# BoxLib-Codes/VARDEN

Hardware: AMD Instinct MI355X
Metric: cells*steps/sec on advance_timestep (higher is better)
Workload: dtype f64; 1 GPU; 3D 256x256x256 single-level variable-density bubble, 1 box(es) of 256^3, MAC+HG projection each step (BASELINE.json configs[1]); parallelism=single GPU, cells=16777216

## Files before the change

### varden_amd/csrc/mg_nd.hip

```cpp
#include "vdn_dev.h"
#include "mg_stop.h"
#include "krylov_wg.h"
#include "krylov_grid.h"
#include <tuple>
#include <algorithm>

struct NLev {
  int n[3]; int PX, PY; long sz;
  double f[3];
  double *phi, *tmp, *b, *res, *sig;
  int dirlo[3], dirhi[3];
  int per[3];
};
DEVI long nidx(const NLev &L, int i, int j, int k) { return (long)(i + 16) + (long)L.PX * ((long)(j + 1) + (long)L.PY * (long)(k + 1)); }
DEVI bool nd_is_dir(const NLev &L, int i, int j, int k) {
  return (i == 0 && L.dirlo[0]) || (i == L.n[0] && L.dirhi[0]) || (j == 0 && L.dirlo[1]) || (j == L.n[1] && L.dirhi[1]) ||
         (k == 0 && L.dirlo[2]) || (k == L.n[2] && L.dirhi[2]);
}
DEVI bool nd_is_shell(const NLev &L, int i, int j, int k, int hm) {
  return ((hm & 1) && i == 0) || ((hm & 2) && i == L.n[0]) || ((hm & 4) && j == 0) || ((hm & 8) && j == L.n[1]) ||
         ((hm & 16) && k == 0) || ((hm & 32) && k == L.n[2]);
}

struct NdW { double w0, w1, w2, w3, w4, w5, w6, w7; int iso; };
DEVI NdW nd_weights(const double f[3]) {
  const double fx = f[0], fy = f[1], fz = f[2];
  const double F = fx + fy + fz;
  NdW W;
  W.w0 = 4.0 * F;
  W.w1 = -4.0 * fx + 2.0 * fy + 2.0 * fz;
  W.w2 = 2.0 * fx - 4.0 * fy + 2.0 * fz;
  W.w3 = -2.0 * fx - 2.0 * fy + fz;
  W.w4 = 2.0 * fx + 2.0 * fy - 4.0 * fz;
  W.w5 = -2.0 * fx + fy - 2.0 * fz;
  W.w6 = fx - 2.0 * fy - 2.0 * fz;
  W.w7 = -F;
// ... 488 lines not shown
  const long sy = C.PX, sz = (long)C.PX * C.PY;
  const double *__restrict__ cp = C.phi;
  long c0 = nidx(C, c00 + (i >> 1), c01 + (j >> 1), c02 + (k0 >> 1));
  double a00 = cp[c0], a10 = cp[c0 + 1], a01 = cp[c0 + sy], a11 = cp[c0 + sy + 1];
  const bool dir_ij = (i == 0 && F.dirlo[0]) || (i == F.n[0] && F.dirhi[0]) || (j == 0 && F.dirlo[1]) || (j == F.n[1] && F.dirhi[1]);
  const double w0 = 1.0 / (double)((1 + oi) * (1 + oj)), w1 = 1.0 / (double)((1 + oi) * (1 + oj) * 2);
  for (int k = k0; k <= k1; k += 2) {
    const double b00 = cp[c0 + sz], b10 = cp[c0 + sz + 1], b01 = cp[c0 + sz + sy], b11 = cp[c0 + sz + sy + 1];
    const long f = nidx(F, i, j, k);
    const double pe = F.phi[f];
    const bool odd_in = k + 1 <= k1;
    const long f2 = f + (long)F.PX * F.PY;
    const double po = odd_in ? F.phi[f2] : 0.0;
    double s = 0.0;
    s = s + a00;
    s = oi ? s + a10 : s;
    s = oj ? s + a01 : s;
    s = (oi && oj) ? s + a11 : s;
    double t = s;
    t = t + b00;
    t = oi ? t + b10 : t;
    t = oj ? t + b01 : t;
    t = (oi && oj) ? t + b11 : t;
    if (!(dir_ij || (k == 0 && F.dirlo[2]) || (k == F.n[2] && F.dirhi[2]))) F.phi[f] = pe + s * w0;
    if (odd_in && !(dir_ij || (k + 1 == F.n[2] && F.dirhi[2]))) F.phi[f2] = po + t * w1;
    a00 = b00; a10 = b10; a01 = b01; a11 = b11; c0 += sz;
  }
}
static void nd_launch_prolong(const NLev &F, const NLev &C, int c00, int c01, int c02) {
  const int nzp = F.n[2] + 1;
  const int kchunk = nzp > 64 ? 16 : (nzp > 16 ? 8 : 2);
  hipLaunchKernelGGL(kk_nd_prolong_m, dim3((F.n[0] + 64) / 64, (F.n[1] + 4) / 4, (nzp + kchunk - 1) / kchunk), dim3(64, 4, 1), 0, ctx().stream, F, C, c00, c01, c02, kchunk);
}
__global__ void kk_nd_coarsen_sigma(NLev F, NLev C) {
  const int i = blockIdx.x * blockDim.x + threadIdx.x;
  const int j = blockIdx.y * blockDim.y + threadIdx.y;
  const int k = blockIdx.z;
  if (i >= C.n[0] || j >= C.n[1] || k >= C.n[2]) return;
  const long sy = F.PX, sz = (long)F.PX * F.PY;
  const long f = nidx(F, 2 * i, 2 * j, 2 * k);
  double s = 0.0;
  #pragma unroll
  for (int c = 0; c < 2; c++)
    #pragma unroll
    for (int b = 0; b < 2; b++)
      #pragma unroll
      for (int a = 0; a < 2; a++) s = s + F.sig[f + a + b * sy + c * sz];
  C.sig[nidx(C, i, j, k)] = s * 0.125;
}

__global__ void __launch_bounds__(1024) kk_nd_bottom(NLev L, double *a, double *b, int nsweeps, double omega, double om1 = 0.0, double om2 = 0.0, int nsp = 0) {
  const int ex = L.n[0] + 3, ey = L.n[1] + 3, ez = L.n[2] + 3;
  const int nx = L.n[0] + 1, ny = L.n[1] + 1, nz = L.n[2] + 1;
  double *src = a, *dst = b;
  for (int s = 0; s < nsweeps; s++) {
    for (int t = threadIdx.x; t < ex * ey * ez; t += blockDim.x) {
      const int i = t % ex - 1, j = (t / ex) % ey - 1, k = t / (ex * ey) - 1;
      int q[3] = { i, j, k }, sidx[3] = { i, j, k }; bool g = false, zero = false;
      for (int d = 0; d < 3; d++) {
        if (L.per[d]) { if (q[d] < 0) { sidx[d] = q[d] + L.n[d]; g = true; } else if (q[d] >= L.n[d]) { sidx[d] = q[d] - L.n[d]; g = true; } }
        else if (q[d] < 0 || q[d] > L.n[d]) { g = true; zero = true; }
      }
      if (g) src[nidx(L, i, j, k)] = zero ? 0.0 : src[nidx(L, sidx[0], sidx[1], sidx[2])];
    }
    __syncthreads();
    for (int t = threadIdx.x; t < nx * ny * nz; t += blockDim.x) {
// ... 326 lines not shown
  G.rev = 0;
  return G;
}
static bool nd_wide_level(const NLev &L) { return sw().nd_pair && L.n[0] >= 127; }
static bool nd_wide_even_level(const NLev &L) { return nd_wide_level(L) && L.n[0] % 2 == 0 && L.n[1] % 2 == 0 && L.n[2] % 2 == 0; }
template <int MODE> static void nd_launch_march(const NLev &L, const double *phi, double *out, double *nrm, int shell_later = 0, int rev = 0, const NLev *pro = nullptr) {
  const int nzp = L.n[2] + 1;
  const int tiles = ((L.n[0] + 62) / 62) * ((L.n[1] + 4) / 4);
  int kchunk = nzp;
  while (kchunk > 8 && tiles * ((nzp + kchunk - 1) / kchunk) < 2048) kchunk = (kchunk + 1) / 2;
  const int nch = (nzp + kchunk - 1) / kchunk;
  if (nd_wide_level(L)) {
    const int rows = 4;
    const bool use_rem = true; const int minwg = 2048, kc_env = 0;
    NdPairGrid G = nd_pair_grid(L, rows, nzp, use_rem, minwg, kc_env);
    G.rev = sw().nd_rev ? rev : 0;
    if (MODE == 0 && pro) {
      const NdCoarse C{ pro->phi, pro->PX, pro->PY, pro->n[0] };
      hipLaunchKernelGGL((kk_nd_march_pair<0, 4, 1>), dim3(G.nmain + G.gyr * G.gz), NBLK, 0, ctx().stream, L, phi, out, nd_cur_omega(), G, nrm, shell_later, C);
      return;
    }
    hipLaunchKernelGGL((kk_nd_march_pair<MODE, 4>), dim3(G.nmain + G.gyr * G.gz), NBLK, 0, ctx().stream, L, phi, out, nd_cur_omega(), G, nrm, shell_later, NdCoarse{ nullptr, 0, 0, 0 });
    return;
  }
  REQUIRE(!pro, "nodal multigrid: the prolonging sweep is the paired march's");
  hipLaunchKernelGGL(kk_nd_march<MODE>, dim3((L.n[0] + 62) / 62, (L.n[1] + 4) / 4, nch), NBLK, 0, ctx().stream, L, phi, out, nd_cur_omega(), kchunk, nrm, shell_later);
}

struct NBox { NLev L; int lo[3]; int hmask = 63; XPlan *hA = nullptr, *hB = nullptr; double *A = nullptr, *B = nullptr; };
struct NDLev { std::vector<NBox> boxes; XPlan *halo_A = nullptr, *halo_B = nullptr, *halo_res = nullptr, *halo_sig = nullptr; int ng[3]; bool flip = false; bool single_box = false; int per[3] = {0, 0, 0};
               int rev = 0;
               bool res_restricted = false;  };
struct NDMG {
  std::vector<NDLev> dlev; std::vector<NLev> tail; int per[3]; double *d_nrm; unsigned pro_levels = 0;
  MgGather g_nodes, g_cells; GBox *d_gb = nullptr;
  double *sendbuf = nullptr, *recvbuf = nullptr;
  MgKrylov kry;
};

__global__ void kk_nd_zero_shell(NLev L, double *a0, double *a1, double *a2) {
  const int u = (int)(blockIdx.x * blockDim.x + threadIdx.x) - 1, v = (int)(blockIdx.y * blockDim.y + threadIdx.y) - 1;
  const int face = blockIdx.z, d = face >> 1, side = face & 1;
  const int da = d == 0 ? 1 : 0, db = d == 2 ? 1 : 2;
  if (u > L.n[da] + 1 || v > L.n[db] + 1) return;
  int q[3]; q[d] = side ? L.n[d] + 1 : -1; q[da] = u; q[db] = v;
  const long c = nidx(L, q[0], q[1], q[2]);
  a0[c] = 0.0; if (a1) a1[c] = 0.0; if (a2) a2[c] = 0.0;
}
static NLev nd_alloc_lev(const int n[3], const double h[3]) {
  NLev L;
  for (int d = 0; d < 3; d++) { L.n[d] = n[d]; L.f[d] = 1.0 / (36.0 * (h[d] * h[d])); L.dirlo[d] = L.dirhi[d] = L.per[d] = 0; }
  L.PX = ((n[0] + 18 + 15) / 16) * 16; L.PY = n[1] + 3; L.sz = (long)L.PX * L.PY * (n[2] + 3);
  double *base = (double *)arena_alloc(sizeof(double) * L.sz * 5);
  L.phi = base; L.tmp = base + L.sz; L.b = base + 2 * L.sz; L.res = base + 3 * L.sz; L.sig = base + 4 * L.sz;
  if (sw().nd_lean && (long)(n[0] + 1) * (n[1] + 1) * (n[2] + 1) >= (1L << 21)) {
    const int m = std::max(n[0], std::max(n[1], n[2])) + 3;
    hipLaunchKernelGGL(kk_nd_zero_shell, dim3((m + 63) / 64, (m + 3) / 4, 6), dim3(64, 4, 1), 0, ctx().stream, L, L.phi, L.tmp, L.res);
    HIPCHK(hipMemsetAsync(L.sig, 0, sizeof(double) * L.sz, ctx().stream));
  } else HIPCHK(hipMemsetAsync(base, 0, sizeof(double) * L.sz * 5, ctx().stream));
  return L;
}
static FV nd_view(const NLev &L, double *p, const int lo[3], int extra ) {
  FV f; f.p = p; f.a0 = lo[0] - 16; f.a1 = lo[1] - 1; f.a2 = lo[2] - 1; f.n0 = L.PX; f.n1 = L.PY; f.n2 = L.n[2] + extra; f.sc = L.sz;
  return f;
}

static void nd_build(NDMG &M, const vdn_multifab *coeffs, const double *dx, const int bc[3][2]) {
// ... 273 lines not shown
  int nl = 0;
  if (dl >= 0) {
    if (!M.tail.empty() && !(ctx().nranks == 1 && M.dlev.back().single_box)) return false;
    for (int m = dl; m < (int)M.dlev.size(); m++) {
      const NDLev &D = M.dlev[m];
      if (!(D.single_box && D.boxes.size() == 1 && (long)(D.ng[0] + 1) * (D.ng[1] + 1) * (D.ng[2] + 1) <= tail_nodes) || nl == ND_TAIL_MAX) return false;
      T.L[nl] = D.boxes[0].L; for (int d = 0; d < 3; d++) T.L[nl].per[d] = D.per[d];
      nl++;
    }
  }
  for (int m = tl; m < (int)M.tail.size(); m++) {
    const NLev &L = M.tail[m];
    if ((long)(L.n[0] + 1) * (L.n[1] + 1) * (L.n[2] + 1) > tail_nodes || nl == ND_TAIL_MAX) return false;
    T.L[nl++] = L;
  }
  if (nl < 2) return false;
  const NLev &B = T.L[nl - 1];
  const int N = std::max(B.n[0], std::max(B.n[1], B.n[2]));
  T.nlev = nl; T.nu1 = P.hg_nu1; T.nu2 = P.hg_nu2; T.nbot = std::max(P.hg_nub, 2 * N * N); T.omega = P.hg_omega; { const NdOm o = nd_om(true, P.hg_nu1); T.om1 = o.om1; T.om2 = o.om2; T.nsp = o.nsp; }
  if (M.kry.w) { hipLaunchKernelGGL(kk_nd_tailcycle_krylov, dim3(1), dim3(1024), 0, ctx().stream, T, nd_krylov_args(M), M.kry.method); T.nbot = 0;  }
  else
  hipLaunchKernelGGL(kk_nd_tailcycle, dim3(1), dim3(1024), 0, ctx().stream, T);
  int m = 0;
  if (dl >= 0) for (int q = dl; q < (int)M.dlev.size(); q++, m++) {
    const int sweeps = (m == nl - 1) ? T.nbot : T.nu1 + T.nu2;
    if (sweeps & 1) { NDLev &D = M.dlev[q]; std::swap(D.boxes[0].L.phi, D.boxes[0].L.tmp); D.flip = !D.flip; }
  }
  for (int q = tl; q < (int)M.tail.size(); q++, m++) {
    const int sweeps = (m == nl - 1) ? T.nbot : T.nu1 + T.nu2;
    if (sweeps & 1) std::swap(M.tail[q].phi, M.tail[q].tmp);
  }
  return true;
}
static void nd_vcycle_d(NDMG &M, int l) {
  const vdn_params &P = ctx().prm;
  NDLev &DL = M.dlev[l];
  if (nd_small_end(M, l, 0)) return;
  const bool last = (l == (int)M.dlev.size() - 1);
  if (last && M.tail.empty() && M.kry.w && DL.single_box && DL.boxes.size() == 1) {
    NBox &B = DL.boxes[0];
    NLev Lp = B.L;
    for (int d = 0; d < 3; d++) Lp.per[d] = DL.per[d];
    nd_krylov_visit(M, Lp, B.L.phi);
    return;
  }
  if (last && M.tail.empty()) { nd_jacobi_d(DL, nd_bottom_sweeps_global(DL)); return; }
  nd_jacobi_d(DL, P.hg_nu1, true);
  nd_residual_d(M, DL, false);
  nd_restrict_down(M, l);
  if (last) nd_vcycle_t(M, 0); else nd_vcycle_d(M, l + 1);
  nd_prolong_smooth(M, l);
}
static long nd_level_nodes(const NDMG &M, int g) {
  const int nd = (int)M.dlev.size();
  if (g < nd) return (long)(M.dlev[g].ng[0] + 1) * (M.dlev[g].ng[1] + 1) * (M.dlev[g].ng[2] + 1);
  const NLev &T = M.tail[g - nd];
  return (long)(T.n[0] + 1) * (T.n[1] + 1) * (T.n[2] + 1);
}
static void nd_cycle_at(NDMG &M, int g) {
  const vdn_params &P = ctx().prm;
  const int nd = (int)M.dlev.size();
  if (g < nd) {
    nd_jacobi_d(M.dlev[g], P.hg_nu1, true);
    nd_residual_d(M, M.dlev[g], false);
    nd_restrict_down(M, g);
    if (g + 1 < nd) nd_vcycle_d(M, g + 1); else nd_vcycle_t(M, 0);
    nd_prolong_up(M, g);
    nd_jacobi_d(M.dlev[g], P.hg_nu2);
    return;
  }
  const int t = g - nd;
  nd_jacobi_t(M.tail[t], P.hg_nu1, true);
  NLev &L = M.tail[t]; NLev &C = M.tail[t + 1];
  nd_fill_nodes(L, L.phi);
  nd_launch_march<1>(L, L.phi, L.res, nullptr);
  nd_fill_nodes(L, L.res);
  hipLaunchKernelGGL(kk_nd_restrict, ng3(C.n[0] + 1, C.n[1] + 1, C.n[2] + 1), NBLK, 0, ctx().stream, L, C);
  nd_vcycle_t(M, t + 1);
  nd_fill_nodes(M.tail[t + 1], M.tail[t + 1].phi);
// ... 65 lines not shown
  g_nd_post[key] = M;
}

struct NdKeep { bool built = false; NDMG M; };
NdKeep *nd_keep_new() { return new NdKeep; }
void nd_keep_free(NdKeep *k) { delete k; }
int nd_solve(NdRequest &q) {
  Prof prof_("hg_multigrid");
  if (ctx().prm.dm == 2) return nd2_solve(q);
  const vdn_params &P = ctx().prm;
  vdn_multifab *rh = q.rh, *phi = q.phi, *add_to = q.add_to; const vdn_multifab *u = q.u; const double *dx = q.dx;
  NdKeep *keep = q.keep; NdFast *fast = q.fast;
  const bool fixed_cycles = q.fixed_cycles > 0;
  REQUIRE(dx && q.bc && q.fixed_cycles >= 0, "nodal multigrid: dx, bc and fixed_cycles >= 0");
  if (fast) REQUIRE(fast->rhohalf && u && u->ng >= 1 && u->nc >= 3 && !keep && !fixed_cycles, "nodal multigrid: the fast path needs rhohalf and u with a ghost cell");
  else REQUIRE(rh && phi && q.coeffs && rh->ng >= 1 && phi->ng >= 1 && q.coeffs->ng >= 1, "nodal multigrid: rh, phi, coeffs need one ghost layer");
  if (u && !fast) REQUIRE(u->ng >= 1 && u->nc >= 3, "nodal multigrid: u needs a ghost cell");
  if (q.rh_is_b) REQUIRE(fixed_cycles && !u && !fast, "nodal multigrid: rh_is_b is the fixed-cycle correction solve's");
  const vdn_multifab *coeffs = fast ? fast->rhohalf : q.coeffs;
  g_nd_iso = nd_isotropic(dx);
  hipStream_t st = ctx().stream;
  size_t mark = arena_mark();
  NDMG M_local;
  NDMG &M = keep ? keep->M : M_local;
  const bool rebuild = !(keep && keep->built);
  if (rebuild) nd_build(M, coeffs, dx, q.bc);
  NDLev &D0 = M.dlev[0];
  if (!fixed_cycles || rebuild) {
    bottom_form_set(1, M.kry.w ? (M.kry.part ? 2 : 1) : 0);
    if (M.kry.w) { const int budget = bottom_budget_begin(1, M.kry.kind, M.kry.maxit); if (M.kry.part) M.kry.budget = budget; }
  }
  if (M.kry.w && (!fixed_cycles || rebuild)) bottom_stats_reset(1);
  M.pro_levels = 0; g_nd_pro_levels = 0;
  if (rebuild) {
  for (size_t b = 0; b < D0.boxes.size(); b++) {
    NLev &L0 = D0.boxes[b].L; const vdn_box &bx = coeffs->vbox[b];
    if (fast) {
      hipLaunchKernelGGL(kk_nd_load_sigma_rho, ng3(L0.n[0] + 2, L0.n[1] + 2, L0.n[2] + 2), NBLK, 0, st, L0, fast->rhohalf->fabs[b], bx.lo[0], bx.lo[1], bx.lo[2]);
    } else
    hipLaunchKernelGGL(kk_nd_load_sigma, ng3(L0.n[0] + 2, L0.n[1] + 2, L0.n[2] + 2), NBLK, 0, st, L0, coeffs->fabs[b], bx.lo[0], bx.lo[1], bx.lo[2]);
  }
  if (fast && D0.halo_sig) xplan_run(D0.halo_sig);
  for (size_t l = 1; l < M.dlev.size(); l++) {
    for (size_t b = 0; b < M.dlev[l].boxes.size(); b++) {
      NLev &C = M.dlev[l].boxes[b].L;
      hipLaunchKernelGGL(kk_nd_coarsen_sigma, ng3(C.n[0], C.n[1], C.n[2]), NBLK, 0, st, M.dlev[l - 1].boxes[b].L, C);
    }
    if (M.dlev[l].halo_sig) xplan_run(M.dlev[l].halo_sig);
  }
  if (!M.tail.empty()) {
    NDLev &DL = M.dlev.back();
    const int nb = (int)M.g_nodes.gb.size();
    for (size_t b = 0; b < DL.boxes.size(); b++) {
      const NLev &F = DL.boxes[b].L;
      hipLaunchKernelGGL(kk_nd_coarsen_sigma_pack, ng3(F.n[0] / 2, F.n[1] / 2, F.n[2] / 2), NBLK, 0, st, F, M.sendbuf, M.g_cells.loc_off[b], F.n[0] / 2, F.n[1] / 2, F.n[2] / 2);
    }
    comm_allgather_dev(M.sendbuf, M.recvbuf, M.g_cells.cnt);
    hipLaunchKernelGGL(kk_nd_unpack, dim3(4, 1, (unsigned)nb), dim3(256), 0, st, M.tail[0], M.tail[0].sig, M.recvbuf, M.d_gb + nb, 0);
    hipLaunchKernelGGL(kk_nd_fill_cells, ng3(M.tail[0].n[0] + 2, M.tail[0].n[1] + 2, M.tail[0].n[2] + 2), NBLK, 0, st, M.tail[0], M.tail[0].sig);
    for (size_t l = 1; l < M.tail.size(); l++) {
      NLev &C = M.tail[l];
      hipLaunchKernelGGL(kk_nd_coarsen_sigma, ng3(C.n[0], C.n[1], C.n[2]), NBLK, 0, st, M.tail[l - 1], C);
      hipLaunchKernelGGL(kk_nd_fill_cells, ng3(C.n[0] + 2, C.n[1] + 2, C.n[2] + 2), NBLK, 0, st, C, C.sig);
    }
  }
  }
// ... 37 lines not shown
    }
    s.conv = true;
  } else {
    const int gn[3] = { M.dlev[0].ng[0], M.dlev[0].ng[1], M.dlev[0].ng[2] };
    s = mg_stop_loop(1, gn, fast && !single && p0max == 0.0, fast && !single, q, bnorm, M.d_nrm,
      [&](bool blind) {
        nd_jacobi_d(M.dlev[0], single ? nd_bottom_sweeps_global(M.dlev[0]) : P.hg_nu1, !single);
        nd_residual_d(M, M.dlev[0], true, !blind);
      },
      [&] {
        if (single) { nd_jacobi_d(M.dlev[0], nd_bottom_sweeps_global(M.dlev[0])); nd_residual_d(M, M.dlev[0], true); }
        else nd_run_cycle(M, 1, [&] { correct(); nd_jacobi_d(M.dlev[0], P.hg_nu1, true); nd_residual_d(M, M.dlev[0], true); });
      },
      [&](int n) {
        nd_run_cycle(M, 8 + 4 * n, [&] {
          for (int c = 0; c < n; c++) { correct(); nd_jacobi_d(M.dlev[0], P.hg_nu1, true); nd_residual_d(M, M.dlev[0], true, false); norm_hist_push(M.d_nrm); }
        });
      },
      [&] { return read_scalar1(M.d_nrm); });
    if (s.overshot) { arena_release(mark); return mg_repeat_unpredicted([&] { return nd_solve(q); }); }
  }
  NDLev &DF = M.dlev[0];
  nd_halo_phi(DF);
  if (fast) fast->phi_view.clear();
  for (size_t b = 0; b < DF.boxes.size(); b++) {
    NLev &L0 = DF.boxes[b].L; const vdn_box &bx = coeffs->vbox[b];
    if (fast) { fast->phi_view.push_back(nd_view(L0, L0.phi, bx.lo, 3)); continue; }
    if (add_to) hipLaunchKernelGGL(kk_nd_store_add, ng3(L0.n[0] + 3, L0.n[1] + 3, L0.n[2] + 3), NBLK, 0, st, L0, phi->fabs[b], add_to->fabs[b], bx.lo[0], bx.lo[1], bx.lo[2]);
    else
    hipLaunchKernelGGL(kk_nd_store, ng3(L0.n[0] + 3, L0.n[1] + 3, L0.n[2] + 3), NBLK, 0, st, L0, phi->fabs[b], bx.lo[0], bx.lo[1], bx.lo[2]);
  }
  q.cycles = s.cycles; q.res0 = bnorm; q.res = s.res;
  g_nd_pro_levels = M.pro_levels;
  if (!keep && !fast) arena_release(mark);
  return s.conv ? 0 : 1;
}

struct UvecArgs { int lo[3], hi[3], ng; int phys[3][2]; double dt, dtinv; int proj_type; };
struct create_uvec_K { FV unew; FV uold; FV rhohalf; FV gp; UvecArgs A;
  __device__ void cell(int i, int j, int k) const {
    const int q[3] = { i, j, k };
    bool g1 = true;
  #pragma unroll
    for (int d = 0; d < 3; d++) if (q[d] < A.lo[d] - 1 || q[d] > A.hi[d] + 1) g1 = false;
    bool wall_plane = false, inlet_plane = false;
  #pragma unroll
    for (int d = 0; d < 3; d++) {
      if (q[d] == A.lo[d] - 1) { int p = A.phys[d][0]; if (p == VDN_SLIP_WALL || p == VDN_NO_SLIP_WALL) wall_plane = true; if (p == VDN_INLET) inlet_plane = true; }
      if (q[d] == A.hi[d] + 1) { int p = A.phys[d][1]; if (p == VDN_SLIP_WALL || p == VDN_NO_SLIP_WALL) wall_plane = true; if (p == VDN_INLET) inlet_plane = true; }
    }
  #pragma unroll
    for (int m = 0; m < 3; m++) {
      double gpv = 0.0;
      if (g1) { gpv = fv_get(gp, i, j, k, m); if (inlet_plane) { gpv = 0.0; fv_at(gp, i, j, k, m) = 0.0; } }
      if (wall_plane) { fv_at(unew, i, j, k, m) = 0.0; continue; }
      if (!g1) continue;
      double v = fv_get(unew, i, j, k, m);
      if (A.proj_type == VDN_PRESSURE_ITERS) v = (v - fv_get(uold, i, j, k, m)) * A.dtinv;
      else if (A.proj_type == VDN_REGULAR_TIMESTEP) v = v + A.dt * gpv / fv_get(rhohalf, i, j, k, 0);
      fv_at(unew, i, j, k, m) = v;
    }
  } };

struct coeffs_K { FV coeffs; FV rhohalf;
  __device__ void cell(int i, int j, int k) const {
    fv_at(coeffs, i, j, k) = 1.0 / fv_get(rhohalf, i, j, k, 0);
// ... 803 lines not shown
```

### varden_amd/csrc/runtime.hip

```cpp
#include "vdn_dev.h"
#include <algorithm>
#include <chrono>
#include <map>
#include <tuple>

static VdnCtx g_ctx;
VdnCtx &ctx() { return g_ctx; }
static thread_local char g_err[1024] = "";

void vdn_set_error(const char *fmt, ...) { va_list ap; va_start(ap, fmt); vsnprintf(g_err, sizeof g_err, fmt, ap); va_end(ap); }
void vdn_fail(const char *fmt, ...) {
  char buf[1024]; va_list ap; va_start(ap, fmt); vsnprintf(buf, sizeof buf, fmt, ap); va_end(ap);
  throw VdnErr(buf);
}

static std::vector<vdn_multifab *> g_temp_mfs;
void arena_reset() {
  dbg_sync(16);
  for (vdn_multifab *m : g_temp_mfs) delete m;
  g_temp_mfs.clear();
  if (sw().arena_poison && g_ctx.arena && g_ctx.arena_peak > 0) HIPCHK(hipMemsetAsync(g_ctx.arena, 0xFF, std::min(g_ctx.arena_peak + (size_t)(64 << 20), g_ctx.arena_bytes), g_ctx.stream));
  g_ctx.arena_off = 0;
  g_ctx.drop_step_caches();
}
// ... 129 lines not shown
Prof::~Prof() { if (on) g_roctx_pop(); }

static Switches g_sw;
const Switches &sw() { static const bool filled = (switches_read(g_sw), true); (void)filled; return g_sw; }
const Switches &sw_live() { sw(); switches_read(g_sw, true); return g_sw; }
extern "C" const char *vdn_build_flavour(void) {
#ifdef VDN_TESTING_BUILD
  return "testing";
#else
  return "release";
#endif
}
extern char **environ;
static void env_warn_unknown() {
  static bool done = false;
  if (done) return;
  done = true;
  for (char **e = environ; e && *e; e++) {
    if (strncmp(*e, "VDN_", 4) != 0 || !strncmp(*e, "VDN_BENCH_", 10) || !strncmp(*e, "VDN_WORKER_", 11)) continue;
    const char *eq = strchr(*e, '=');
    const size_t len = eq ? (size_t)(eq - *e) : strlen(*e);
    bool known = false;
    for (const SwitchInfo &s : switch_table) if (strlen(s.name) == len && !strncmp(s.name, *e, len)) known = true;
    if (!strncmp(*e, "VDN_LIB_FLAVOUR", 15)) continue;
    if (!known) fprintf(stderr, "varden_amd: warning: environment variable %.*s is not a switch of this library (vdn_debug_switches lists them)\n", (int)len, *e);
#ifndef VDN_TESTING_BUILD
    else fprintf(stderr, "varden_amd: note: %.*s is set but this is the release build: launch-form switches are compiled out (libvarden_amd_testing.so reads them)\n", (int)len, *e);
#endif
  }
}
#ifdef VDN_TESTING_BUILD
unsigned nd_last_prolong_levels();
extern "C" unsigned vdn_nd_prolong_fused_levels(void) { return nd_last_prolong_levels(); }
#endif
extern "C" const char *vdn_debug_switches(void) {
  static std::string out;
#ifndef VDN_TESTING_BUILD
  if (out.empty()) out = "release build: the switches below are compiled out, every launch form is the default one (libvarden_amd_testing.so reads them)\n";
#endif
  if (out.find(std::string(switch_table[0].name) + " ") == std::string::npos) for (const SwitchInfo &s : switch_table) { const char *v = switch_raw(s); out += s.name; out += v ? std::string(" = ") + v : std::string(" (unset)"); out += ": "; out += s.doc; out += "\n"; }
  return out.c_str();
}

bool g_capturing_now();
__global__ void k_publish(double *host_view, const double *dev, int n, unsigned long long seq) {
  if ((int)threadIdx.x < n) host_view[threadIdx.x] = dev[threadIdx.x];
  __syncthreads();
  if (threadIdx.x == 0) { __threadfence_system(); *reinterpret_cast<volatile unsigned long long *>(host_view + 64) = seq; }
}
const double *read_scalars(const double *dev, int n) {
  VdnCtx &c = g_ctx;
  REQUIRE(n >= 1 && n <= 64, "read_scalars: 1..64 values");
  static unsigned long long seq = 0;
  const bool poll = sw().poll >= 0 ? sw().poll != 0 : c.nranks == 1;
  ++seq;
  dbg_sync(8);
  hipLaunchKernelGGL(k_publish, dim3(1), dim3(64), 0, c.stream, c.h_scal_dev, dev, n, seq);
  if (poll && !g_capturing_now()) {
    volatile unsigned long long *flag = reinterpret_cast<volatile unsigned long long *>(c.h_scal + 64);
    for (unsigned long spins = 1;; spins++) {
      if (*flag == seq) { __sync_synchronize(); return c.h_scal; }
      __builtin_ia32_pause();
      if ((spins & 0xfff) == 0) {
        const hipError_t q = hipStreamQuery(c.stream);
        if (q == hipSuccess) break;
        if (q != hipErrorNotReady) HIPCHK(q);
// ... 740 lines not shown
```

### varden_amd/csrc/vdn_switches.h

```cpp
#pragma once
#include <algorithm>
#include <cstddef>
#include <cstdlib>
#include <cstring>

#define VDN_SWITCHES(X) \
  X(testing, "VDN_TESTING", STR, nullptr, "1: allows VDN_RCCL_LIB (the test transport of tests/fake_rccl); nothing else") \
  X(rccl_lib, "VDN_RCCL_LIB", STR, nullptr, "path of a library that stands in for librccl -- honoured only with VDN_TESTING=1 and the test double's handshake") \
  X(force_packed, "VDN_FORCE_PACKED", LIVE, 0, "1: box-to-box copies of one rank go through the packed per-peer buffers (device memcpy for send/recv); 2: through a 1-rank RCCL communicator (one-GPU rehearsal of the N > 1 transport)") \
  X(arena_poison, "VDN_ARENA_POISON", SET, false, "1: every byte handed back to the arena is overwritten with NaNs (a read of an entry nobody wrote fails the next solve)") \
  X(arena_chunk, "VDN_ARENA_CHUNK_MB", MB, (size_t)1024 << 20, "size of the physical chunks mapped into the arena's address range (default 1024)") \
  X(field_chunk, "VDN_FIELD_CHUNK_MB", MB, (size_t)64 << 20, "size of the pooled physical chunks behind the state fields (default 64)") \
  X(field_vmm, "VDN_FIELD_VMM", ON, true, "0: every state field is one hipMalloc block (rounds 1-5) instead of pooled chunks mapped into its own address range") \
  X(mlcc_trace, "VDN_MLCC_TRACE", SET, false, "1: the composite cell-centred solve prints its residual at every FAC iteration (stderr)") \
  X(keep_off, "VDN_KEEP_OFF", INT, 0, "mask of kept-descriptor families rebuilt at every call: 1 generic sets, 2 create_umac_grown, 4 composite cell-centred solve, 8 nodal prolongation") \
  X(sync_points, "VDN_SYNC_POINTS", INT, 0, "mask of points that synchronise the device (race hunting): 1 after every batched launch, 2 after every staged upload, 4 after every exchange, 8 before a scalar read-back, 16 at arena_reset, 32 after launch_cells") \
  X(phase_hash, "VDN_PHASE_HASH", SET, false, "1: advance_timestep prints a checksum of its fields at every phase boundary (stderr)") \
  X(no_roctx, "VDN_NO_ROCTX", PRESENT, false, "do not bind the roctx library (no bl_prof ranges)") \
  X(poll, "VDN_POLL", INT, -1, "scalar read-back: 1 spin on the pinned sequence number, 0 hipStreamSynchronize; default: spin on one rank, synchronise on several") \
  X(no_graphs, "VDN_NO_GRAPHS", PRESENT, false, "launch every multigrid cycle eagerly instead of replaying its hipGraph") \
  X(no_slope_cache, "VDN_NO_SLOPE_CACHE", PRESENT, false, "velocity mkflux recomputes the slopes of uold that velpred computed in the same step") \
  X(no_force_reuse, "VDN_NO_FORCE_REUSE", SET, false, "1: every forcing term is computed where the reference computes it (advance_premac AND velocity_advance, ...)") \
  X(slopes_march, "VDN_SLOPES_MARCH", ON, true, "0: the per-cell slopes kernel instead of the k-marching one") \
  X(godunov_batch, "VDN_GODUNOV_BATCH", SET, false, "1: the descriptor (box-batched) Godunov kernels also on a level of one box") \
  X(godunov_plain, "VDN_GODUNOV_PLAIN", PRESENT, false, "the face-centred one-thread-per-cell Godunov kernels of round 1 (the fused marches' bit-for-bit reference, and their fallback where they refuse the field layouts)") \
  X(god_segw, "VDN_GOD_SEGW", ON, true, "0: the box-batched fused Godunov marches use full-width (64 x 8) tiles for every box") \
  X(god_p2, "VDN_GOD_P2", ON, true, "0: the fused marches divide by dx also where every dx is a power of two (default there: scale by 1/dx, the same doubles)") \
  X(fused_kchunks, "VDN_FUSED_KCHUNKS", MIN1, 0, "k-chunks of the fused marches (default: the count that fills the last round of workgroups best)") \
  X(god_update, "VDN_GOD_UPDATE", ON, true, "0: update_3d as its own pass instead of inside the fused mkflux march") \
  X(gsrb_pair, "VDN_GSRB_PAIR", ON, true, "0: one cell per thread in the colour passes / residuals of wide levels instead of the 2 x 2 pair form") \
  X(mac_split, "VDN_MAC_SPLIT", ON, true, "0: the finest level of macproject's one-level solve stays interleaved (kk_cc_gsrb_rho_pair) instead of stored by colour (kk_cc_gsrb_rho_split)") \
  X(mac_split_min, "VDN_MAC_SPLIT_MIN", INT, 1<<23, "fewest cells (of this rank's boxes together) of a level stored by colour (default 2^23)") \
  X(nd_rev, "VDN_ND_REV", ON, true, "0: every march of a nodal level walks its tiles in the same order (default: consecutive marches alternate)") \
  X(mac_slab, "VDN_MAC_SLAB", INT, -1, "planes per slab of the time-skewed schedule of the split level's passes (cc_split_run; default: ~200 MB of pass traffic, at most half the level); 0: whole-level launches") \
  X(mac_umax, "VDN_MAC_UMAX", ON, true, "0: max |umac| by its own pass (kk_macmax) instead of inside macproject's velocity update (kk_mkumac_rho_max)") \
  X(mac_kflip, "VDN_MAC_KFLIP", ON, true, "0: both colour passes of a sweep walk the planes upwards (default: the second colour downwards; paired and split passes of the cell-centred multigrid)") \
  X(cc_halo_faces, "VDN_CC_HALO_FACES", ON, true, "0: the cell-centred multigrid exchanges the whole ghost shell instead of the faces only") \
  X(overlap, "VDN_OVERLAP", INT, -1, "halo exchange of multigrid passes next to interior work: 1 always, 0 never, default: when a plan has a remote peer and the box is large") \
  X(mg_agglom, "VDN_MG_AGGLOM", INT, 0, "box width below which a multi-box multigrid level is gathered into one box (default: 64 across ranks, 128 where every box is this rank's)") \
  X(mg_restrict_fused, "VDN_MG_RESTRICT_FUSED", ON, true, "0: cell-centred residual and restriction as two passes") \
  X(mg_tailcycle, "VDN_MG_TAILCYCLE", ON, true, "0: the smallest levels launch by launch instead of one single-workgroup cycle") \
  X(mg_prolong_fused, "VDN_MG_PROLONG_FUSED", ON, true, "0: cell-centred prolongation as its own pass instead of inside the first post-smoothing colour pass") \
  X(mg_lds, "VDN_MG_LDS", ON, true, "0: the 16^3..64^3 cell-centred levels launch by launch instead of the LDS-tiled down / up kernels") \
  X(mac_stored_beta, "VDN_MAC_STORED_BETA", SET, false, "1: the finest MAC level reads stored face coefficients instead of recomputing them from rho") \
  X(mac_fast, "VDN_MAC_FAST", ON, true, "0: macproject with its rh / phi / beta multifabs as the reference has them") \
  X(hg_fast, "VDN_HG_FAST", ON, true, "0: hgproject with its rh / phi / coeffs multifabs as the reference has them") \
  X(nd_pair, "VDN_ND_PAIR", ON, true, "0: one node per lane in the nodal march instead of the pair form") \
  X(nd_lean, "VDN_ND_LEAN", ON, true, "0: whole-array zero fills of the big nodal levels instead of shell-only") \
  X(nd_restrict_fused, "VDN_ND_RESTRICT_FUSED", ON, true, "0: nodal residual and full weighting as two passes") \
  X(nd_prolong_fused, "VDN_ND_PROLONG_FUSED", ON, true, "0: nodal prolongation as a pass of its own instead of inside the first post-smoothing march") \
  X(ndf_pair, "VDN_NDF_PAIR", ON, true, "0: one node per lane in the box-batched nodal march of the composite solve") \
  X(ndm_iface_faces, "VDN_NDM_IFACE_FACES", ON, true, "0: interface interpolation of the composite nodal solve over whole boxes instead of box faces") \
  X(ndm_prolong8, "VDN_NDM_PROLONG8", ON, true, "0: correction interpolation with a thread per fine node instead of per coarse node") \
  X(ndm_neg, "VDN_NDM_NEG", SET, false, "1: the composite nodal solve copies -res into the correction's right-hand side instead of loading it directly") \
  X(fb_faces, "VDN_FB_FACES", ON, true, "0: the ghost exchanges of the composite cell-centred solve fill edges and corners too") \
  X(mlcc_rho, "VDN_MLCC_RHO", ON, true, "0: the composite MAC solve reads stored face coefficients on its finest level too") \
  X(god_narrow, "VDN_GOD_NARROW", ON, true, "0: the remainder tile column of the fused mkflux + update march in full 64-lane tiles instead of narrow segments (kk_mk_F_mn)") \
  X(keep_sets, "VDN_KEEP_SETS", ON, true, "0: the descriptor arrays of the inter-level operators and composite solves are rebuilt and uploaded at every call") \
  X(kept_bound, "VDN_KEPT_BOUND", INT, 0, "n > 0: the kept descriptor tables hold at most n entries each (default 4096 / 64 / 512): the eviction paths in a test") \
  X(mlcc_glue, "VDN_MLCC_GLUE", ON, true, "0: the level-0 correction of the composite MAC solve stored and added in separate passes") \
  X(mlcc_fuse1, "VDN_MLCC_FUSE1", ON, true, "0: the composite MAC solve's finest-level residual and first colour pass as two launches") \
  X(batch_yz, "VDN_BATCH_YZ", ON, true, "0: no (j,k) / (i,k) tiles for thin ranges in the box-batched kernels") \
  X(batch_ppw, "VDN_BATCH_PPW", MIN1, 0, "planes per workgroup of the light box-batched kernels (default 8)") \
  X(batch_flat, "VDN_BATCH_FLAT", ON, true, "0: no flattened (i,j) plane mapping for badly filling tiles") \
  X(batch_chunk, "VDN_BATCH_CHUNK", ON, true, "0: box-batched workgroups take strided instead of contiguous plane chunks")

static inline bool sw_read_ON(const char *e, bool) { return !(e && atoi(e) == 0); }
static inline bool sw_read_SET(const char *e, bool) { return e && atoi(e) != 0; }
static inline bool sw_read_PRESENT(const char *e, bool) { return e != nullptr; }
static inline int sw_read_INT(const char *e, int dflt) { return e ? atoi(e) : dflt; }
static inline int sw_read_MIN1(const char *e, int dflt) { return e ? std::max(1, atoi(e)) : dflt; }
static inline size_t sw_read_MB(const char *e, size_t dflt) { const long v = e ? atol(e) : 0; return v > 0 ? (size_t)v << 20 : dflt; }
static inline const char *sw_read_STR(const char *e, const char *) { return e; }
static inline int sw_read_LIVE(const char *e, int dflt) { return sw_read_INT(e, dflt); }

struct Switches {
// ... 23 lines not shown
```

Measured before the change: 675.5 million cells*steps/s.

## Fuse mid-size nodal multigrid levels into LDS-tiled down and up kernels

For single-box, non-periodic nodal levels of 16 to 64 cells per side, the two pre-smoothing sweeps, the residual and the full-weighting restriction run in one kernel on an 8^3 tile with a halo held in shared memory. The prolongation and post-smoothing sweep run in a second LDS kernel. This replaces several small launches per level with two, cutting launch overhead and global-memory round trips on levels too small to fill the GPU. The cost is redundant halo recomputation and 1024-thread blocks with large LDS footprints, and the path only applies when nu1=2 and nu2=1.

```diff
diff --git a/varden_amd/csrc/mg_nd.hip b/varden_amd/csrc/mg_nd.hip
--- a/varden_amd/csrc/mg_nd.hip
+++ b/varden_amd/csrc/mg_nd.hip
@@ -2,6 +2,7 @@
 #include "mg_stop.h"
 #include "krylov_wg.h"
 #include "krylov_grid.h"
+#include "nd_lds_plan.h"
 #include <tuple>
 #include <algorithm>
 
@@ -556,6 +557,151 @@
   const int kchunk = nzp > 64 ? 16 : (nzp > 16 ? 8 : 2);
   hipLaunchKernelGGL(kk_nd_prolong_m, dim3((F.n[0] + 64) / 64, (F.n[1] + 4) / 4, (nzp + kchunk - 1) / kchunk), dim3(64, 4, 1), 0, ctx().stream, F, C, c00, c01, c02, kchunk);
 }
+#define ND_LDS_NT 1024
+DEVI void nd_lds_gather(const double *__restrict__ ph, int e, int c, const double *__restrict__ sgb, int se, int sc, double p[3][3][3], double sg[2][2][2]) {
+  #pragma unroll
+  for (int k = 0; k < 3; k++)
+    #pragma unroll
+    for (int j = 0; j < 3; j++)
+      #pragma unroll
+      for (int i = 0; i < 3; i++) p[k][j][i] = ph[c + (i - 1) + (j - 1) * e + (k - 1) * e * e];
+  #pragma unroll
+  for (int k = 0; k < 2; k++)
+    #pragma unroll
+    for (int j = 0; j < 2; j++)
+      #pragma unroll
+      for (int i = 0; i < 2; i++) sg[k][j][i] = sgb[sc + i + j * se + k * se * se];
+}
+__global__ void __launch_bounds__(ND_LDS_NT) kk_nd_lds_down(NLev L, NLev C, double om1, double om2) {
+  constexpr int E = ND_LDS_BOX, E3 = E * E * E, S = ND_LDS_SIG, S3 = S * S * S;
+  __shared__ double pa[E3], pb[E3], sgb[S3];
+  const int ta[3] = { (int)blockIdx.x, (int)blockIdx.y, (int)blockIdx.z };
+  const int x0 = nd_lds_box_lo(ta[0]), y0 = nd_lds_box_lo(ta[1]), z0 = nd_lds_box_lo(ta[2]);
+  const int tid = threadIdx.x;
+  for (int t = tid; t < S3; t += ND_LDS_NT) {
+    const int i = x0 - 1 + t % S, j = y0 - 1 + (t / S) % S, k = z0 - 1 + t / (S * S);
+    const bool in = i >= 0 && i < L.n[0] && j >= 0 && j < L.n[1] && k >= 0 && k < L.n[2];
+    sgb[t] = in ? L.sig[nidx(L, i, j, k)] : 0.0;
+  }
+  for (int t = tid; t < E3; t += ND_LDS_NT) pb[t] = 0.0;
+  const NdW W = nd_weights(L.f);
+  __syncthreads();
+  for (int t = tid; t < E3; t += ND_LDS_NT) {
+    const int bi = t % E, bj = (t / E) % E, bk = t / (E * E);
+    const int i = x0 + bi, j = y0 + bj, k = z0 + bk;
+    double v = 0.0;
+    if (i >= 0 && i <= L.n[0] && j >= 0 && j <= L.n[1] && k >= 0 && k <= L.n[2]) {
+      double p[3][3][3], sg[2][2][2];
+      #pragma unroll
+      for (int c = 0; c < 3; c++)
+        #pragma unroll
+        for (int b = 0; b < 3; b++)
+          #pragma unroll
+          for (int a = 0; a < 3; a++) p[c][b][a] = 0.0;
+      #pragma unroll
+      for (int c = 0; c < 2; c++)
+        #pragma unroll
+        for (int b = 0; b < 2; b++)
+          #pragma unroll
+          for (int a = 0; a < 2; a++) sg[c][b][a] = sgb[(bi + a) + (bj + b) * S + (bk + c) * S * S];
+      const double p0 = p[1][1][1];
+      double Kp, diag; nd_stencil(W, p, sg, Kp, diag);
+      if (!nd_is_dir(L, i, j, k) && diag != 0.0) v = p0 + om1 * ((L.b[nidx(L, i, j, k)] - Kp) / diag);
+    }
+    pa[t] = v;
+  }
+  __syncthreads();
+  {
+    constexpr int R = E - 2;
+    const NdLdsRange ox = nd_lds_own_fine(L.n[0], ta[0]), oy = nd_lds_own_fine(L.n[1], ta[1]), oz = nd_lds_own_fine(L.n[2], ta[2]);
+    for (int t = tid; t < R * R * R; t += ND_LDS_NT) {
+      const int bi = 1 + t % R, bj = 1 + (t / R) % R, bk = 1 + t / (R * R);
+      const int i = x0 + bi, j = y0 + bj, k = z0 + bk;
+      if (!(i >= 0 && i <= L.n[0] && j >= 0 && j <= L.n[1] && k >= 0 && k <= L.n[2])) continue;
+      double p[3][3][3], sg[2][2][2];
+      const int c = bi + bj * E + bk * E * E;
+      nd_lds_gather(pa, E, c, sgb, S, bi + bj * S + bk * S * S, p, sg);
+      const double p0 = p[1][1][1];
+      const long g = nidx(L, i, j, k);
+      double Kp, diag; nd_stencil(W, p, sg, Kp, diag);
+      double v = p0;
+      if (!nd_is_dir(L, i, j, k) && diag != 0.0) v = p0 + om2 * ((L.b[g] - Kp) / diag);
+      pb[c] = v;
+      if (i >= ox.lo && i <= ox.hi && j >= oy.lo && j <= oy.hi && k >= oz.lo && k <= oz.hi) L.phi[g] = v;
+    }
+  }
+  __syncthreads();
+  {
+    constexpr int R = E - 2;
+    const NdLdsRange rx = nd_lds_resid(L.n[0], ta[0]), ry = nd_lds_resid(L.n[1], ta[1]), rz = nd_lds_resid(L.n[2], ta[2]);
+    for (int t = tid; t < R * R * R; t += ND_LDS_NT) {
+      const int bi = 2 + t % R, bj = 2 + (t / R) % R, bk = 2 + t / (R * R);
+      const int i = x0 + bi, j = y0 + bj, k = z0 + bk;
+      const int c = bi + bj * E + bk * E * E;
+      double r = 0.0;
+      if (i >= 0 && i <= min(L.n[0], rx.hi) && j >= 0 && j <= min(L.n[1], ry.hi) && k >= 0 && k <= min(L.n[2], rz.hi) && !nd_is_dir(L, i, j, k)) {
+        double p[3][3][3], sg[2][2][2];
+        nd_lds_gather(pb, E, c, sgb, S, bi + bj * S + bk * S * S, p, sg);
+        double Kp, diag; nd_stencil(W, p, sg, Kp, diag);
+        r = L.b[nidx(L, i, j, k)] - Kp;
+      }
+      pa[c] = r;
+    }
+  }
+  __syncthreads();
+  {
+    const NdLdsRange cx = nd_lds_own_coarse(L.n[0], ta[0]), cy = nd_lds_own_coarse(L.n[1], ta[1]), cz = nd_lds_own_coarse(L.n[2], ta[2]);
+    constexpr int Q = ND_LDS_T / 2 + 1;
+    for (int t = tid; t < Q * Q * Q; t += ND_LDS_NT) {
+      const int qi = t % Q, qj = (t / Q) % Q, qk = t / (Q * Q);
+      const int i = cx.lo + qi, j = cy.lo + qj, k = cz.lo + qk;
+      if (i > cx.hi || j > cy.hi || k > cz.hi) continue;
+      double s = 0.0;
+      if (!nd_is_dir(C, i, j, k)) s = nd_fw27(pa + (3 + 2 * qi) + (3 + 2 * qj) * E + (3 + 2 * qk) * E * E, E, E * E);
+      const long cn = nidx(C, i, j, k);
+      C.b[cn] = s * 0.125;
+      C.phi[cn] = 0.0;
+    }
+  }
+}
+__global__ void __launch_bounds__(ND_LDS_NT) kk_nd_lds_up(NLev L, NLev C, double omega) {
+  constexpr int E = ND_LDS_UBOX, E3 = E * E * E, S = ND_LDS_USIG, S3 = S * S * S;
+  __shared__ double ph[E3], sgb[S3];
+  const int ta[3] = { (int)blockIdx.x, (int)blockIdx.y, (int)blockIdx.z };
+  const int x0 = nd_lds_ubox_lo(ta[0]), y0 = nd_lds_ubox_lo(ta[1]), z0 = nd_lds_ubox_lo(ta[2]);
+  const int tid = threadIdx.x;
+  for (int t = tid; t < S3; t += ND_LDS_NT) {
+    const int i = x0 + t % S, j = y0 + (t / S) % S, k = z0 + t / (S * S);
+    const bool in = i >= 0 && i < L.n[0] && j >= 0 && j < L.n[1] && k >= 0 && k < L.n[2];
+    sgb[t] = in ? L.sig[nidx(L, i, j, k)] : 0.0;
+  }
+  for (int t = tid; t < E3; t += ND_LDS_NT) {
+    const int i = x0 + t % E, j = y0 + (t / E) % E, k = z0 + t / (E * E);
+    double v = 0.0;
+    if (i >= 0 && i <= L.n[0] && j >= 0 && j <= L.n[1] && k >= 0 && k <= L.n[2]) {
+      v = L.phi[nidx(L, i, j, k)];
+      if (!nd_is_dir(L, i, j, k)) v = v + nd_interp8(C, C.phi, i >> 1, j >> 1, k >> 1, i & 1, j & 1, k & 1);
+    }
+    ph[t] = v;
+  }
+  const NdW W = nd_weights(L.f);
+  __syncthreads();
+  const NdLdsRange ox = nd_lds_own_fine(L.n[0], ta[0]), oy = nd_lds_own_fine(L.n[1], ta[1]), oz = nd_lds_own_fine(L.n[2], ta[2]);
+  constexpr int R = ND_LDS_T + 1;
+  for (int t = tid; t < R * R * R; t += ND_LDS_NT) {
+    const int bi = 1 + t % R, bj = 1 + (t / R) % R, bk = 1 + t / (R * R);
+    const int i = x0 + bi, j = y0 + bj, k = z0 + bk;
+    if (i > ox.hi || j > oy.hi || k > oz.hi) continue;
+    double p[3][3][3], sg[2][2][2];
+    nd_lds_gather(ph, E, bi + bj * E + bk * E * E, sgb, S, (bi - 1) + (bj - 1) * S + (bk - 1) * S * S, p, sg);
+    const double p0 = p[1][1][1];
+    const long g = nidx(L, i, j, k);
+    double Kp, diag; nd_stencil(W, p, sg, Kp, diag);
+    double v = p0;
+    if (!nd_is_dir(L, i, j, k) && diag != 0.0) v = p0 + omega * ((L.b[g] - Kp) / diag);
+    L.tmp[g] = v;
+  }
+}
 __global__ void kk_nd_coarsen_sigma(NLev F, NLev C) {
   const int i = blockIdx.x * blockDim.x + threadIdx.x;
   const int j = blockIdx.y * blockDim.y + threadIdx.y;
@@ -948,7 +1094,7 @@
                int rev = 0;
                bool res_restricted = false;  };
 struct NDMG {
-  std::vector<NDLev> dlev; std::vector<NLev> tail; int per[3]; double *d_nrm; unsigned pro_levels = 0;
+  std::vector<NDLev> dlev; std::vector<NLev> tail; int per[3]; double *d_nrm; unsigned pro_levels = 0, lds_levels = 0;
   MgGather g_nodes, g_cells; GBox *d_gb = nullptr;
   double *sendbuf = nullptr, *recvbuf = nullptr;
   MgKrylov kry;
@@ -1288,6 +1434,17 @@
   }
   return true;
 }
+static bool nd_lds_level(const NDMG &M, int l) {
+  const vdn_params &P = ctx().prm;
+  if (!sw().mg_lds || l < 1 || l + 1 >= (int)M.dlev.size() || ctx().nranks != 1 || P.hg_nu1 != 2 || P.hg_nu2 != 1 || M.per[0] || M.per[1] || M.per[2]) return false;
+  const NDLev &D = M.dlev[l], &DC = M.dlev[l + 1];
+  if (!(D.single_box && D.boxes.size() == 1 && !D.halo_A && !D.halo_B && !D.halo_res && !(D.per[0] || D.per[1] || D.per[2]) && DC.single_box && DC.boxes.size() == 1)) return false;
+  const NBox &B = D.boxes[0];
+  for (int d = 0; d < 3; d++) if (!nd_lds_extent_ok(B.L.n[d]) || B.lo[d] != 0 || DC.boxes[0].L.n[d] * 2 != B.L.n[d]) return false;
+  return true;
+}
+static unsigned g_nd_lds_levels = 0;
+unsigned nd_last_lds_levels() { return g_nd_lds_levels; }
 static void nd_vcycle_d(NDMG &M, int l) {
   const vdn_params &P = ctx().prm;
   NDLev &DL = M.dlev[l];
@@ -1301,6 +1458,19 @@
     return;
   }
   if (last && M.tail.empty()) { nd_jacobi_d(DL, nd_bottom_sweeps_global(DL)); return; }
+  if (nd_lds_level(M, l)) {
+    const dim3 g((unsigned)nd_lds_tiles(DL.boxes[0].L.n[0]), (unsigned)nd_lds_tiles(DL.boxes[0].L.n[1]), (unsigned)nd_lds_tiles(DL.boxes[0].L.n[2]));
+    const NdOm om = nd_om(true, P.hg_nu1);
+    hipLaunchKernelGGL(kk_nd_lds_down, g, dim3(ND_LDS_NT), 0, ctx().stream, DL.boxes[0].L, M.dlev[l + 1].boxes[0].L, om.at(0), om.at(1));
+    M.lds_levels |= 1u << l;
+    nd_vcycle_d(M, l + 1);
+    nd_halo_phi(M.dlev[l + 1]);
+    NDLev &D = M.dlev[l];
+    hipLaunchKernelGGL(kk_nd_lds_up, g, dim3(ND_LDS_NT), 0, ctx().stream, D.boxes[0].L, M.dlev[l + 1].boxes[0].L, P.hg_omega);
+    std::swap(D.boxes[0].L.phi, D.boxes[0].L.tmp);
+    D.flip = !D.flip;
+    return;
+  }
   nd_jacobi_d(DL, P.hg_nu1, true);
   nd_residual_d(M, DL, false);
   nd_restrict_down(M, l);
@@ -1432,6 +1602,7 @@
   }
   if (M.kry.w && (!fixed_cycles || rebuild)) bottom_stats_reset(1);
   M.pro_levels = 0; g_nd_pro_levels = 0;
+  M.lds_levels = 0; g_nd_lds_levels = 0;
   if (rebuild) {
   for (size_t b = 0; b < D0.boxes.size(); b++) {
     NLev &L0 = D0.boxes[b].L; const vdn_box &bx = coeffs->vbox[b];
@@ -1535,6 +1706,7 @@
   }
   q.cycles = s.cycles; q.res0 = bnorm; q.res = s.res;
   g_nd_pro_levels = M.pro_levels;
+  g_nd_lds_levels = M.lds_levels;
   if (!keep && !fast) arena_release(mark);
   return s.conv ? 0 : 1;
 }
diff --git a/varden_amd/csrc/nd_lds_plan.h b/varden_amd/csrc/nd_lds_plan.h
--- /dev/null
+++ b/varden_amd/csrc/nd_lds_plan.h
@@ -0,0 +1,30 @@
+#pragma once
+#if defined(__HIPCC__)
+#define ND_LDS_FN __host__ __device__ inline
+#else
+#define ND_LDS_FN inline
+#endif
+
+#define ND_LDS_T 8
+#define ND_LDS_NMIN 16
+#define ND_LDS_NMAX 64
+#define ND_LDS_BOX 13
+#define ND_LDS_SIG 14
+#define ND_LDS_UBOX 11
+#define ND_LDS_USIG 10
+
+struct NdLdsRange { int lo, hi; };
+
+ND_LDS_FN bool nd_lds_extent_ok(int n) { return n % ND_LDS_T == 0 && n >= ND_LDS_NMIN && n <= ND_LDS_NMAX; }
+ND_LDS_FN int nd_lds_tiles(int n) { return n / ND_LDS_T; }
+ND_LDS_FN bool nd_lds_last(int n, int a) { return a == n / ND_LDS_T - 1; }
+ND_LDS_FN NdLdsRange nd_lds_own_fine(int n, int a) { return NdLdsRange{ ND_LDS_T * a, nd_lds_last(n, a) ? n : ND_LDS_T * a + ND_LDS_T - 1 }; }
+ND_LDS_FN NdLdsRange nd_lds_own_coarse(int n, int a) { return NdLdsRange{ (ND_LDS_T / 2) * a, nd_lds_last(n, a) ? n / 2 : (ND_LDS_T / 2) * a + ND_LDS_T / 2 - 1 }; }
+ND_LDS_FN int nd_lds_box_lo(int a) { return ND_LDS_T * a - 3; }
+ND_LDS_FN int nd_lds_sig_lo(int a) { return ND_LDS_T * a - 4; }
+ND_LDS_FN int nd_lds_ubox_lo(int a) { return ND_LDS_T * a - 1; }
+ND_LDS_FN int nd_lds_usig_lo(int a) { return ND_LDS_T * a - 1; }
+ND_LDS_FN NdLdsRange nd_lds_sweep1(int a) { return NdLdsRange{ ND_LDS_T * a - 3, ND_LDS_T * a + 9 }; }
+ND_LDS_FN NdLdsRange nd_lds_sweep2(int a) { return NdLdsRange{ ND_LDS_T * a - 2, ND_LDS_T * a + 8 }; }
+ND_LDS_FN NdLdsRange nd_lds_resid(int n, int a) { return NdLdsRange{ ND_LDS_T * a - 1, nd_lds_last(n, a) ? ND_LDS_T * a + 8 : ND_LDS_T * a + 7 }; }
+ND_LDS_FN NdLdsRange nd_lds_resbox(int a) { return NdLdsRange{ ND_LDS_T * a - 1, ND_LDS_T * a + 9 }; }
diff --git a/varden_amd/csrc/runtime.hip b/varden_amd/csrc/runtime.hip
--- a/varden_amd/csrc/runtime.hip
+++ b/varden_amd/csrc/runtime.hip
@@ -185,6 +185,8 @@
 #ifdef VDN_TESTING_BUILD
 unsigned nd_last_prolong_levels();
 extern "C" unsigned vdn_nd_prolong_fused_levels(void) { return nd_last_prolong_levels(); }
+unsigned nd_last_lds_levels();
+extern "C" unsigned vdn_nd_lds_levels(void) { return nd_last_lds_levels(); }
 #endif
 extern "C" const char *vdn_debug_switches(void) {
   static std::string out;
diff --git a/varden_amd/csrc/vdn_switches.h b/varden_amd/csrc/vdn_switches.h
--- a/varden_amd/csrc/vdn_switches.h
+++ b/varden_amd/csrc/vdn_switches.h
@@ -41,7 +41,7 @@
   X(mg_restrict_fused, "VDN_MG_RESTRICT_FUSED", ON, true, "0: cell-centred residual and restriction as two passes") \
   X(mg_tailcycle, "VDN_MG_TAILCYCLE", ON, true, "0: the smallest levels launch by launch instead of one single-workgroup cycle") \
   X(mg_prolong_fused, "VDN_MG_PROLONG_FUSED", ON, true, "0: cell-centred prolongation as its own pass instead of inside the first post-smoothing colour pass") \
-  X(mg_lds, "VDN_MG_LDS", ON, true, "0: the 16^3..64^3 cell-centred levels launch by launch instead of the LDS-tiled down / up kernels") \
+  X(mg_lds, "VDN_MG_LDS", ON, true, "0: the 16^3..64^3-cell levels of both multigrids (cell-centred and nodal) launch by launch instead of the LDS-tiled down / up kernels") \
   X(mac_stored_beta, "VDN_MAC_STORED_BETA", SET, false, "1: the finest MAC level reads stored face coefficients instead of recomputing them from rho") \
   X(mac_fast, "VDN_MAC_FAST", ON, true, "0: macproject with its rh / phi / beta multifabs as the reference has them") \
   X(hg_fast, "VDN_HG_FAST", ON, true, "0: hgproject with its rh / phi / coeffs multifabs as the reference has them") \
```

Result: faster. 694.0 million cells*steps/s (median of 6 runs) (+2.7%).
